# NickTravers/NeuralNetworkLibrary

Measured on AMD Instinct MI355X. Metric: ResNet-34 224x224 training throughput (Learner.train1minibatch, fwd+loss+bwd+optimizer), higher is better.
Workload: dtype f32; 1 GPU; DogsCats ResNet-34 classifier, 224x224, bs=64 per GPU, SGD momentum 0.9, fp32; global_batch=64, image_size=224, parallelism=dp1

## Files before the change

include/nnl.h:

```cpp
#ifndef NNL_H_
#define NNL_H_

#include <stddef.h>
#include <stdint.h>

#ifdef __cplusplus
extern "C" {
#endif

typedef enum {
  NNL_OK = 0,
  NNL_ERR_INVALID_ARG = -1,
  NNL_ERR_HIP = -2,
  NNL_ERR_UNSUPPORTED = -3,
  NNL_ERR_WORKSPACE = -4
} nnl_status_t;

int nnl_version(void);
const char* nnl_last_error(void);
int nnl_reload_env(void);

enum { NNL_PROF_CONV_FWD = 0, NNL_PROF_CONV_DGRAD = 1, NNL_PROF_CONV_WGRAD = 2, NNL_PROF_EMBDOT = 3,
       NNL_PROF_TABULAR = 4, NNL_PROF_RETINA_LOSS = 5, NNL_PROF_LSTM = 6, NNL_PROF_SOFTMAX_CE = 7,
       NNL_PROF_ELEMENTWISE = 8, NNL_PROF_GEMM = 9, NNL_PROF_OPTIM = 10, NNL_PROF_KINDS = 11 };
// ... 13 lines not shown
                       float* dU, float* dM, float* dbu, float* dbi, int64_t n, int64_t n_user,
                       int64_t n_item, int64_t D, int has_range, float lo, float hi, void* workspace, size_t workspace_bytes, void* stream);

typedef struct {
  int32_t N, H, W, C;
  int32_t K, R, S;
  int32_t stride, pad;
  int32_t P, Q;
} nnl_conv_geom_t;

size_t nnl_conv2d_fwd_workspace_bytes(const nnl_conv_geom_t* g);
int64_t nnl_conv2d_tile_counters(void);
int nnl_conv2d_fwd(const float* x, const float* w, const float* bias, float* y, const nnl_conv_geom_t* g,
                   int relu, void* workspace, size_t workspace_bytes, int32_t* tile_counters, float* bn_partials,
                   const float* bn_pivot, int32_t* bn_rows, void* stream);
int nnl_conv2d_fwd_add_up2(const float* x, const float* w, const float* bias, const float* small, float* y,
                           const nnl_conv_geom_t* g, void* stream);
int nnl_upsample2_bwd(const float* dy, float* dsmall, int64_t N, int64_t h, int64_t w, int64_t C, void* stream);
int nnl_conv2d_weight_transpose(const float* w, float* wt, int K, int R, int S, int C, void* stream);
typedef struct {
  const float* w;
  float* wt;
  int32_t K, RS, C, first_tile;
} nnl_wt_desc_t;
int nnl_conv2d_weight_transpose_multi(const nnl_wt_desc_t* desc, const int32_t* tile_tensor, int64_t n_tiles,
                                      double total_elems, void* stream);
size_t nnl_conv2d_dgrad_workspace_bytes(const nnl_conv_geom_t* g);
int nnl_conv2d_dgrad(const float* dy, const float* wt, float* dx, const nnl_conv_geom_t* g, const float* addend,
                     void* workspace, size_t workspace_bytes, int32_t* tile_counters, void* stream);
typedef struct {
// ... 37 lines not shown
int nnl_bn_fwd(const float* x, const float* gamma, const float* beta, const float* residual, float* y,
               float* save_mean, float* save_invstd, float* running_mean, float* running_var, int64_t rows,
               int64_t C, float eps, float momentum, int training, int relu, int64_t* num_batches_tracked,
               uint32_t* relu_mask, const float* ext_partials, int64_t ext_rows, const float* ext_pivot, float* pivot_out,
               void* workspace, size_t workspace_bytes, void* stream);
int nnl_bn_bwd(const float* dy, const float* y, const uint32_t* relu_mask, const float* x, const float* gamma,
               const float* mean, const float* invstd, float* dx, float* dres, float* dgamma, float* dbeta, int64_t rows,
               int64_t C, int training, int relu, void* workspace, size_t workspace_bytes, void* stream);

int nnl_bn_relu_maxpool_supported(int64_t C);
int nnl_bn_relu_maxpool_fwd(const float* x, const float* gamma, const float* beta, float* y, uint8_t* idx, float* save_mean,
                            float* save_invstd, float* save_scale, float* save_shift, float* running_mean, float* running_var,
                            int64_t N, int64_t H, int64_t W, int64_t C, int64_t P, int64_t Q, int ks, int stride, int pad, float eps,
                            float momentum, int training, int64_t* num_batches_tracked, void* workspace, size_t workspace_bytes,
                            void* stream);
int nnl_bn_relu_maxpool_bwd(const float* dpool, const float* y, const uint8_t* idx, const float* x, const float* gamma,
                            const float* beta, const float* mean, const float* invstd, const float* scale, const float* shift,
                            float* dx, float* dgamma, float* dbeta,
                            int64_t N, int64_t H, int64_t W, int64_t C, int64_t P, int64_t Q, int ks, int stride, int pad,
                            int training, void* workspace, size_t workspace_bytes, void* stream);

int nnl_debug_bn_plan(int64_t rows, int64_t C, int64_t N, int64_t H, int64_t W, int64_t P, int64_t Q, int32_t* out10);

int nnl_bn_sync_stats(const float* x, float* stats, int64_t rows, int64_t C, void* workspace, size_t workspace_bytes,
                      void* stream);
int nnl_bn_sync_fwd(const float* x, const float* all_stats, int world, const float* gamma, const float* beta,
                    const float* residual, float* y, float* save_mean, float* save_invstd, float* running_mean,
                    float* running_var, int64_t rows, int64_t C, float eps, float momentum, int relu,
                    int64_t* num_batches_tracked, uint32_t* relu_mask, void* workspace, size_t workspace_bytes, void* stream);
int nnl_bn_sync_bwd_reduce(const float* dy, const float* y, const uint32_t* relu_mask, const float* x, const float* mean,
// ... 239 lines not shown
```

neuralnetworklibrary_amd/_lib.py:

```python
import ctypes as C
import os

import torch

_HERE = os.path.dirname(os.path.abspath(__file__))
LIB_PATH = os.environ.get('NNL_LIB_PATH') or os.path.join(_HERE, 'libnnl_hip.so')

if not os.path.exists(LIB_PATH):
    raise ImportError(
        f"{LIB_PATH} not found: build it with `python -c 'import __graft_entry__ as g; g.build()'` "
        "(or `make -C neuralnetworklibrary_amd/csrc`). There is no CPU fallback for the HIP hot path.")

lib = C.CDLL(LIB_PATH)

c_p = C.c_void_p
i32, i64, f32, f64 = C.c_int32, C.c_int64, C.c_float, C.c_double
sz = C.c_size_t


class ConvGeom(C.Structure):
    _fields_ = [('N', i32), ('H', i32), ('W', i32), ('C', i32), ('K', i32), ('R', i32), ('S', i32),
                ('stride', i32), ('pad', i32), ('P', i32), ('Q', i32)]


# ... 21 lines not shown
    'nnl_conv2d_fwd_pre': (C.c_int, [c_p, c_p, c_p, c_p, C.POINTER(ConvGeom), C.c_int, c_p, sz, c_p, c_p, c_p, C.POINTER(i32), c_p, c_p]),
    'nnl_conv2d_dgrad_pre': (C.c_int, [c_p, c_p, c_p, C.POINTER(ConvGeom), c_p, c_p, sz, c_p, c_p, c_p]),
    'nnl_debug_conv_wino_workspace_bytes': (sz, [C.c_int] * 5),
    'nnl_debug_conv_wino_fwd': (C.c_int, [c_p] * 6 + [sz, c_p, C.c_long, c_p, c_p] + [C.c_int] * 7 + [c_p]),
    'nnl_debug_conv_wino2_workspace_bytes': (sz, [C.c_int] * 5),
    'nnl_debug_conv_wino2_fwd': (C.c_int, [c_p] * 6 + [sz, c_p, C.c_long, c_p, c_p] + [C.c_int] * 7 + [c_p]),
    'nnl_debug_conv_plan_times': (C.c_int, [C.c_int] * 5 + [C.POINTER(C.c_double)]),
    'nnl_debug_route_record': (C.c_int, [C.c_int]),
    'nnl_debug_route_collect': (C.c_int, [C.c_char_p, sz]),
    'nnl_conv2d_fwd': (C.c_int, [c_p, c_p, c_p, c_p, C.POINTER(ConvGeom), C.c_int, c_p, sz, c_p, c_p, c_p, C.POINTER(i32), c_p]),
    'nnl_conv2d_weight_transpose': (C.c_int, [c_p, c_p, C.c_int, C.c_int, C.c_int, C.c_int, c_p]),
    'nnl_conv2d_weight_transpose_multi': (C.c_int, [c_p, c_p, i64, f64, c_p]),
    'nnl_conv2d_dgrad': (C.c_int, [c_p, c_p, c_p, C.POINTER(ConvGeom), c_p, c_p, sz, c_p, c_p]),
    'nnl_conv2d_wgrad_workspace_bytes': (sz, [C.POINTER(ConvGeom)]),
    'nnl_conv2d_wgrad': (C.c_int, [c_p, c_p, c_p, C.POINTER(ConvGeom), c_p, sz, c_p]),
    'nnl_colsum_workspace_bytes': (sz, [i64, i64]),
    'nnl_colsum': (C.c_int, [c_p, c_p, i64, i64, c_p, sz, c_p]),
    'nnl_relu_gate_colsum': (C.c_int, [c_p, c_p, c_p, c_p, i64, i64, c_p, sz, c_p]),
    'nnl_conv2d_fwd_add_up2': (C.c_int, [c_p, c_p, c_p, c_p, c_p, C.POINTER(ConvGeom), c_p]),
    'nnl_upsample2_bwd': (C.c_int, [c_p, c_p, i64, i64, i64, i64, c_p]),
    'nnl_act_gate_colsum': (C.c_int, [c_p, c_p, c_p, c_p, i64, i64, C.c_int, c_p, sz, c_p]),
    'nnl_maxpool2d_fwd': (C.c_int, [c_p, c_p, c_p, i64, i64, i64, i64, i64, i64, C.c_int, C.c_int, C.c_int, c_p]),
    'nnl_maxpool2d_bwd': (C.c_int, [c_p, c_p, c_p, i64, i64, i64, i64, i64, i64, C.c_int, C.c_int, C.c_int, c_p]),
    'nnl_sum_tensors': (C.c_int, [c_p, C.c_int, c_p, i64, c_p]),
    'nnl_bn_relu_maxpool_supported': (C.c_int, [i64]),
    'nnl_bn_relu_maxpool_fwd': (C.c_int, [c_p, c_p, c_p, c_p, c_p, c_p, c_p, c_p, c_p, c_p, c_p, i64, i64, i64, i64, i64, i64,
                                          C.c_int, C.c_int, C.c_int, f32, f32, C.c_int, c_p, c_p, sz, c_p]),
    'nnl_bn_relu_maxpool_bwd': (C.c_int, [c_p, c_p, c_p, c_p, c_p, c_p, c_p, c_p, c_p, c_p, c_p, c_p, c_p, i64, i64, i64, i64, i64, i64,
                                          C.c_int, C.c_int, C.c_int, C.c_int, c_p, sz, c_p]),
    'nnl_concat_pool_fwd': (C.c_int, [c_p, c_p, c_p, i64, i64, i64, c_p]),
    'nnl_concat_pool_bwd': (C.c_int, [c_p, c_p, c_p, i64, i64, i64, c_p]),
    'nnl_gconv2d_fwd': (C.c_int, [c_p, c_p, c_p, c_p, i64, i64, i64, i64, i64, i64, C.c_int, C.c_int, C.c_int, C.c_int, c_p]),
    'nnl_gconv2d_dgrad': (C.c_int, [c_p, c_p, c_p, i64, i64, i64, i64, i64, i64, C.c_int, C.c_int, C.c_int, c_p]),
    'nnl_gconv2d_workspace_bytes': (sz, [i64, i64, i64, i64, i64, i64, C.c_int, C.c_int, C.c_int]),
    'nnl_gconv2d_wgrad': (C.c_int, [c_p, c_p, c_p, c_p, sz, i64, i64, i64, i64, i64, i64, C.c_int, C.c_int, C.c_int, c_p]),
    'nnl_se_squeeze': (C.c_int, [c_p, c_p, i64, i64, i64, c_p]),
    'nnl_se_excite_fwd': (C.c_int, [c_p, c_p, c_p, c_p, i64, i64, i64, c_p]),
    'nnl_se_excite_bwd': (C.c_int, [c_p, c_p, c_p, c_p, c_p, c_p, c_p, i64, i64, i64, c_p]),
    'nnl_se_squeeze_bwd': (C.c_int, [c_p, c_p, i64, i64, i64, c_p]),
    'nnl_bbox_decode': (C.c_int, [c_p, c_p, c_p, i64, i64, i64, c_p, c_p, f32, f32, f32, c_p, c_p, c_p, c_p, c_p, c_p]),
    'nnl_bbox_decode_window': (C.c_int, [c_p, c_p, c_p, i64, i64, i64, c_p, c_p, f32, f32, f32, f32, f32, c_p, c_p, c_p, c_p, c_p, c_p]),
    'nnl_nms_workspace_bytes': (sz, [i64, i64]),
# ... 142 lines not shown
```

neuralnetworklibrary_amd/csrc/batchnorm.hip:

```cpp
#include "nnl_common.h"

namespace {

typedef float f32x4 __attribute__((ext_vector_type(4)));

template <int VEC> struct VecT;
template <> struct VecT<4> { typedef f32x4 type; };
template <> struct VecT<1> { typedef float type; };

template <int VEC> __device__ __forceinline__ float vget(const typename VecT<VEC>::type& v, int i);
template <> __device__ __forceinline__ float vget<4>(const f32x4& v, int i) { return v[i]; }
template <> __device__ __forceinline__ float vget<1>(const float& v, int i) { return v; }
template <int VEC> __device__ __forceinline__ void vset(typename VecT<VEC>::type& v, int i, float x);
template <> __device__ __forceinline__ void vset<4>(f32x4& v, int i, float x) { v[i] = x; }
template <> __device__ __forceinline__ void vset<1>(float& v, int i, float x) { v = x; }

constexpr int kBlock = 256;
constexpr int kMaxRowBlocks = 1024;
constexpr float kCentreAbove = 16.f;
constexpr int kFinLanes = 64;

struct Shape {
  int L;
  int rpb;
// ... 799 lines not shown
  NNL_CHECK_ARG(P == (H + 2 * pad - ks) / stride + 1 && Q == (W + 2 * pad - ks) / stride + 1, "%s: P/Q do not match", who);
  NNL_CHECK_ARG(bnpool_ok(C), "%s: C=%ld needs C %% 4 == 0 and C/4 dividing 256", who, C);
  NNL_CHECK_ARG(N * H * W * C < (1L << 31) * 4, "%s: tensor too large", who);
  return NNL_OK;
}

}

extern "C" int nnl_bn_relu_maxpool_supported(int64_t C) { return bnpool_ok(C) ? 1 : 0; }

extern "C" int nnl_bn_relu_maxpool_fwd(const float* x, const float* gamma, const float* beta, float* y, uint8_t* idx,
                                       float* save_mean, float* save_invstd, float* save_scale, float* save_shift,
                                       float* running_mean, float* running_var, int64_t N, int64_t H, int64_t W, int64_t C,
                                       int64_t P, int64_t Q, int ks, int stride, int pad, float eps, float momentum, int training,
                                       int64_t* num_batches_tracked, void* workspace, size_t workspace_bytes, void* stream) {
  NNL_TRY(check_stem_geometry("bn_relu_maxpool_fwd", N, H, W, C, P, Q, ks, stride, pad));
  NNL_CHECK_ARG(x && y && idx && save_mean && save_invstd && save_scale && save_shift, "bn_relu_maxpool_fwd: null pointer");
  NNL_CHECK_ARG(training || (running_mean && running_var), "bn_relu_maxpool_fwd: eval mode needs running statistics");
  const long rows = (long)N * H * W, CG = C / 4;
  Workspace ws;
  NNL_TRY(bind_workspace(workspace, workspace_bytes, rows, C, "bn_relu_maxpool_fwd", ws));
  hipStream_t s = (hipStream_t)stream;
  NnlProfScope prof(NNL_PROF_ELEMENTWISE, s, (double)rows * C * (training ? 8.0 : 4.0) + (double)N * P * Q * C * 5.0);
  const ChannelStats cs{gamma, beta, save_mean, save_invstd, running_mean, running_var, save_scale, save_shift,  nullptr,
                         nullptr, num_batches_tracked, eps, momentum};
  NNL_TRY(launch_channel_affine(x, ws.part, cs, rows, C, training, s));
  const long total = (long)N * P * Q * CG;
  hipLaunchKernelGGL(bnpool_fwd_kernel, dim3((unsigned)nnl_cdiv(total, kBlock)), dim3(kBlock), 0, s, x, save_scale, save_shift, y, idx,
                     (int)N, (int)H, (int)W, (int)CG, (int)P, (int)Q, ks, stride, pad);
  NNL_CHECK_LAUNCH();
  return NNL_OK;
}

extern "C" int nnl_bn_relu_maxpool_bwd(const float* dpool, const float* y, const uint8_t* idx, const float* x, const float* gamma,
                                       const float* beta, const float* mean, const float* invstd, const float* scale,
                                       const float* shift, float* dx, float* dgamma, float* dbeta, int64_t N,
                                       int64_t H, int64_t W, int64_t C, int64_t P, int64_t Q, int ks, int stride, int pad,
                                       int training, void* workspace, size_t workspace_bytes, void* stream) {
  NNL_TRY(check_stem_geometry("bn_relu_maxpool_bwd", N, H, W, C, P, Q, ks, stride, pad));
  NNL_CHECK_ARG(dpool && idx && x && mean && invstd && scale && shift && dx, "bn_relu_maxpool_bwd: null pointer");
  const long rows = (long)N * H * W;
// ... 105 lines not shown
```

neuralnetworklibrary_amd/csrc/conv2d.hip:

```cpp
#include "igemm_kernels.h"
#include "igemm_taps.h"
#include "split_plan.h"
#include "wino.h"
#include "igemm_wgrad.h"
#include "igemm_wgrad2d.h"

#ifdef NNL_TAPS_TIMING
static void* g_wgrad_dbg = nullptr;
extern "C" void* nnl_debug_wgrad_stamps(void) { return g_wgrad_dbg; }
#endif

namespace {

int check_geom(const nnl_conv_geom_t* g, const char* who) {
  if (!g) return nnl_set_error(NNL_ERR_INVALID_ARG, "%s: null geometry", who);
  if (g->N <= 0 || g->H <= 0 || g->W <= 0 || g->C <= 0 || g->K <= 0 || g->R <= 0 || g->S <= 0 || g->stride <= 0 ||
      g->pad < 0)
    return nnl_set_error(NNL_ERR_INVALID_ARG, "%s: non-positive dimension", who);
  if (g->H + 2L * g->pad < g->R || g->W + 2L * g->pad < g->S)
    return nnl_set_error(NNL_ERR_INVALID_ARG, "%s: the %d x %d filter is larger than the padded input (%d x %d, pad %d)", who, g->R, g->S,
                         g->H, g->W, g->pad);
  const int P = (g->H + 2 * g->pad - g->R) / g->stride + 1, Q = (g->W + 2 * g->pad - g->S) / g->stride + 1;
  if (P != g->P || Q != g->Q || P <= 0 || Q <= 0)
    return nnl_set_error(NNL_ERR_INVALID_ARG, "%s: P,Q=(%d,%d) do not match the geometry (%d,%d)", who, g->P, g->Q, P, Q);
// ... 1017 lines not shown
  if (wgrad_wino_ok(g)) {
    const WgradPlan wp = plan_wgrad_wino(g);
    nnl_prof_exec_frac(1.0 / 1.5);
    int st2 = launch_wgrad_wino(dy, x, (float*)workspace, g, wp, s);
    if (st2) return st2;
    const long n4 = (long)g->K * 3 * (g->C / 4);
    NNL_ROUTE("wgrad_wino1d_finish");
    hipLaunchKernelGGL(wino_wgrad_finish_kernel, dim3((unsigned)nnl_cdiv(n4, 32L)), dim3(256), 0, s, (const float*)workspace, dw, n4,
                       g->C / 4, wp.splits, (long)g->K * 12 * (g->C / 4));
    NNL_CHECK_LAUNCH();
    return NNL_OK;
  }
  return launch_wgrad_direct(p, plan_wgrad(p.Mc, p.Nc, p.Kp), (float*)workspace, dw, s);
}

extern "C" size_t nnl_colsum_workspace_bytes(int64_t rows, int64_t cols) {
  if (rows <= 0 || cols <= 0) return 0;
  return (size_t)colsum_chunks(rows) * cols * sizeof(float);
}

extern "C" int nnl_act_gate_colsum(const float* dy, const float* y, float* g, float* colsum, int64_t rows, int64_t cols, int act,
                                   void* workspace, size_t workspace_bytes, void* stream) {
  NNL_CHECK_ARG(dy && y && g && rows > 0 && cols > 0 && cols < (1L << 30), "act_gate_colsum: bad argument");
  NNL_CHECK_ARG(act == 1 || act == 2, "act_gate_colsum: act must be 1 (ReLU) or 2 (sigmoid)");
  if (colsum != nullptr && (workspace == nullptr || workspace_bytes < nnl_colsum_workspace_bytes(rows, cols)))
    return nnl_set_error(NNL_ERR_WORKSPACE, "act_gate_colsum: workspace too small");
  hipStream_t s = (hipStream_t)stream;
  NnlProfScope prof(NNL_PROF_ELEMENTWISE, s, 12.0 * rows * cols);
  const int nchunk = colsum_chunks(rows);
  const long rpc = nnl_cdiv(nnl_cdiv(rows, nchunk), 4) * 4;
// ... 75 lines not shown
```

neuralnetworklibrary_amd/ops.py:

```python
import collections
import contextlib
import ctypes
import os
import weakref

import numpy as np
import torch

from . import _lib
from ._lib import check, lib, ptr, require_cuda, stream

__all__ = ['mse_loss', 'bce_with_logits', 'fbeta', 'scaled_sigmoid', 'embdotbias', 'index_error_flag', 'raise_if_index_error', 'conv2d', 'to_nhwc', 'from_nhwc', 'linear', 'bn_act', 'concat_pool2d', 'TabularPlan', 'tab_embed_concat', 'embedding_renorm_drop', 'retina_loss', 'image_aug', 'grouped_conv2d', 'se_excite']

_ERR_FLAGS = {}


def _flags(device):
    key = (device.type, device.index)
    if key not in _ERR_FLAGS:
        _ERR_FLAGS[key] = torch.zeros(2, dtype=torch.int32, device=device)
    return _ERR_FLAGS[key]


def index_error_flag(device):
# ... 565 lines not shown
        dxn += shortcut.view_as(dxn)
    give = st.give_slot
    if give is not None and not give.closed and st.c_in == g.C:
        give.tensor = dxn
        return None
    return from_nhwc(dxn[..., :st.c_in] if st.c_in != g.C else dxn)


def _conv_wgrad(st, xn, dy4, g4, K):
    dst = st.grad_dst
    if dst is not None and st.uses is not None and st.uses[0] == 1 and dst.dim() == 4 and g4.K == K and st.c_in == g4.C \
            and dst.permute(0, 2, 3, 1).is_contiguous() and tuple(dst.shape) == (g4.K, g4.C, g4.R, g4.S):
        dwn = dst.permute(0, 2, 3, 1)
    else:
        dwn = torch.empty((g4.K, g4.R, g4.S, g4.C), dtype=torch.float32, device=dy4.device)
    wsb = int(lib.nnl_conv2d_wgrad_workspace_bytes(g4))
    ws = _workspace(wsb, dy4.device, floor=True)
    check(lib.nnl_conv2d_wgrad(ptr(xn), ptr(dy4), ptr(dwn), g4, ptr(ws), wsb, stream()))
    dw = from_nhwc(dwn[:K, :, :, :st.c_in])
    wshape, wstride = st.w_layout
    if (g4.R == 1 and g4.S == 1 and wshape == tuple(dw.shape) and wstride != tuple(dw.stride()) and dw.is_contiguous(memory_format=torch.channels_last)
            and wstride[1] == 1 and wstride[0] == dw.shape[1]):
        dw = dw.as_strided(wshape, wstride)
    return dw


def _conv_bias_grad(dy4, g4, K):
    rows = g4.N * g4.P * g4.Q
    db_full = torch.empty(g4.K, dtype=torch.float32, device=dy4.device)
    cb = int(lib.nnl_colsum_workspace_bytes(rows, g4.K))
    cws = _workspace(cb, dy4.device, floor=True)
    check(lib.nnl_colsum(ptr(dy4), ptr(db_full), rows, g4.K, ptr(cws), cb, stream()))
    return db_full[:K]


class _Conv2d(torch.autograd.Function):

    @staticmethod
    def forward(ctx, x, weight, bias, stride, pad, relu, slot=None, bn_pivot=None, give_slot=None):
        require_cuda(x, weight, bias)
        xn, wn, b, g, y = _conv_operands(x, weight, bias, stride, pad)
        N, K = g.N, g.K
        ctx.st = _conv_state(x, weight, bias, g, relu, slot, give_slot)
        wsb = int(lib.nnl_conv2d_fwd_workspace_bytes(g))
        ws = _workspace(wsb, x.device)
        part, rows = None, _lib.i32(0)
        if bn_pivot is not None:
            part = torch.empty(((N * g.P * g.Q + 63) // 64) * K * 2, dtype=torch.float32, device=x.device)
        u = (_OPEN or _CLOSED).wino(wn.data_ptr(), 0, g)
        check(lib.nnl_conv2d_fwd_pre(ptr(xn), ptr(wn), ptr(b), ptr(y), g, int(relu), ptr(ws), wsb, ptr(_tile_counters(x.device) if wsb else None),
                                     ptr(part), ptr(bn_pivot), ctypes.byref(rows) if part is not None else None, ptr(u), stream()))
        if part is None or rows.value == 0:
            part = torch.empty(0, dtype=torch.float32, device=x.device)
        else:
            part = part[:rows.value * K * 2]
        ctx.mark_non_differentiable(part)
        ctx.set_materialize_grads(False)
        ctx.save_for_backward(xn, wn, y if relu else None)
        return from_nhwc(y), part

    @staticmethod
    def backward(ctx, dy, _dpart=None):
        xn, wn, y = ctx.saved_tensors
        return _conv_backward(ctx.st, xn, wn, y, dy, ctx.needs_input_grad[:3]) + (None,) * 6


# ... 328 lines not shown
        return from_nhwc(y)

    @staticmethod
    def backward(ctx, dy):
        (idx,) = ctx.saved_tensors
        N, H, W, C, P, Q, ksize, stride, pad = ctx.cfg
        dyn = to_nhwc(dy.float())
        dx = torch.empty(N, H, W, C, dtype=torch.float32, device=dy.device)
        check(lib.nnl_maxpool2d_bwd(ptr(dyn), ptr(idx), ptr(dx), N, H, W, C, P, Q, ksize, stride, pad, stream()))
        return from_nhwc(dx), None, None, None, None


class _BNReLUMaxPool(torch.autograd.Function):

    @staticmethod
    def forward(ctx, x, gamma, beta, running_mean, running_var, training, momentum, eps, nbt, ksize, stride, pad):
        require_cuda(x, gamma, beta)
        xn = to_nhwc(x.float())
        N, H, W, C = xn.shape
        P, Q = (H + 2 * pad - ksize) // stride + 1, (W + 2 * pad - ksize) // stride + 1
        dev = x.device
        y = torch.empty(N, P, Q, C, dtype=torch.float32, device=dev)
        idx = torch.empty(N, P, Q, C, dtype=torch.uint8, device=dev)
        stats = torch.empty(4, C, dtype=torch.float32, device=dev)
        wsb = int(lib.nnl_bn_workspace_bytes(N * H * W, C))
        ws = _workspace(wsb, dev)
        check(lib.nnl_bn_relu_maxpool_fwd(ptr(xn), ptr(gamma), ptr(beta), ptr(y), ptr(idx), ptr(stats[0]), ptr(stats[1]),
                                          ptr(stats[2]), ptr(stats[3]), ptr(running_mean), ptr(running_var), N, H, W, C, P, Q,
                                          ksize, stride, pad, float(eps), float(momentum), int(training), ptr(nbt), ptr(ws), wsb,
                                          stream()))
        ctx.save_for_backward(xn, idx, gamma, beta, stats, y)
        ctx.cfg = (N, H, W, C, P, Q, ksize, stride, pad, training)
        return from_nhwc(y)

    @staticmethod
    def backward(ctx, dy):
        xn, idx, gamma, beta, stats, y = ctx.saved_tensors
        N, H, W, C, P, Q, ksize, stride, pad, training = ctx.cfg
        dyn = to_nhwc(dy.float())
        dx = torch.empty_like(xn)
        dgamma = torch.empty(C, dtype=torch.float32, device=xn.device) if gamma is not None else None
        dbeta = torch.empty(C, dtype=torch.float32, device=xn.device) if gamma is not None else None
        wsb = int(lib.nnl_bn_workspace_bytes(N * H * W, C))
        ws = _workspace(wsb, xn.device)
        check(lib.nnl_bn_relu_maxpool_bwd(ptr(dyn), ptr(y), ptr(idx), ptr(xn), ptr(gamma), ptr(beta), ptr(stats[0]), ptr(stats[1]),
                                          ptr(stats[2]), ptr(stats[3]), ptr(dx), ptr(dgamma), ptr(dbeta), N, H, W, C, P, Q, ksize, stride, pad,
                                          int(training), ptr(ws), wsb, stream()))
        return (from_nhwc(dx), dgamma, dbeta) + (None,) * 9


def conv_bn_relu_maxpool(conv, bn, pool, x):
    k, s, p = pool.kernel_size, pool.stride, pool.padding
    fuse = (x.is_cuda and isinstance(pool, torch.nn.MaxPool2d) and all(isinstance(v, int) for v in (k, s, p))
            and pool.dilation == 1 and not pool.ceil_mode and not pool.return_indices and 2 * p <= k and k * k <= 255
            and not (bn.training and getattr(bn, 'nnl_sync', None) is not None)
            and (bn.running_mean is not None or bn.training)
            and not (bn.training and bn.track_running_stats and bn.momentum is None)
            and bool(lib.nnl_bn_relu_maxpool_supported(bn.num_features)))
    if not fuse:
        return pool(conv_bn_act(conv, bn, x, relu=True))
    y = conv(x)
    training, momentum, nbt, rmean, rvar = _bn_mode(bn)
    return _BNReLUMaxPool.apply(y, bn.weight, bn.bias, rmean, rvar, training, momentum, bn.eps, nbt, k, s, p)


def maxpool2d(x, ksize=3, stride=2, pad=1, ceil_mode=False):
    return _MaxPool2d.apply(x, int(ksize), int(stride), int(pad), bool(ceil_mode))


def _gconv_check(x_shape, w_shape, stride, pad, groups):
    if len(x_shape) != 4 or len(w_shape) != 4:
        raise NotImplementedError('grouped_conv2d: x %s and weight %s must be 4-D' % (tuple(x_shape), tuple(w_shape)))
    C, (K, Cg, R, S) = x_shape[1], w_shape
    if R != S or R not in (1, 3):
        raise NotImplementedError('grouped_conv2d: kernel_size %dx%d is not supported (1x1 or 3x3)' % (R, S))
    if stride not in (1, 2):
        raise NotImplementedError('grouped_conv2d: stride %r is not supported (1 or 2)' % (stride,))
    if pad not in (0, 1) or pad > R // 2:
# ... 841 lines not shown
```

Baseline: 5540 images/s.

## Add dedicated 7x7 stem conv kernels with fused BN statistics epilogue

Adds a specialized MFMA kernel for the 7x7 stride-2 stem convolution (C padded to 4, K multiple of 64), plus a slab-based wgrad kernel with a reduction pass. The forward kernel can emit per-channel BN partial sums, and the fused BN+ReLU+maxpool path now consumes those partials instead of re-reading the conv output to compute statistics. The goal is to replace the generic conv path for the stem and remove one full pass over the large stem activation. This adds complexity: a pivot tensor cached on the BN module, a skip during graph capture, and a dedicated code path whose numerics may differ slightly.

```diff
diff --git a/include/nnl.h b/include/nnl.h
--- a/include/nnl.h
+++ b/include/nnl.h
@@ -51,6 +51,12 @@
 int nnl_conv2d_fwd(const float* x, const float* w, const float* bias, float* y, const nnl_conv_geom_t* g,
                    int relu, void* workspace, size_t workspace_bytes, int32_t* tile_counters, float* bn_partials,
                    const float* bn_pivot, int32_t* bn_rows, void* stream);
+int nnl_stem7_supported(const nnl_conv_geom_t* g);
+int nnl_stem7_fwd(const float* x, const float* w, const float* bias, float* y, const nnl_conv_geom_t* g, int relu, float* bn_partials,
+                  const float* bn_pivot, int32_t* bn_rows, void* stream);
+size_t nnl_stem7_wgrad_workspace_bytes(const nnl_conv_geom_t* g);
+int nnl_stem7_wgrad(const float* x, const float* dy, float* dw, const nnl_conv_geom_t* g, void* workspace, size_t workspace_bytes,
+                    void* stream);
 int nnl_conv2d_fwd_add_up2(const float* x, const float* w, const float* bias, const float* small, float* y,
                            const nnl_conv_geom_t* g, void* stream);
 int nnl_upsample2_bwd(const float* dy, float* dsmall, int64_t N, int64_t h, int64_t w, int64_t C, void* stream);
@@ -118,6 +124,12 @@
                             int64_t N, int64_t H, int64_t W, int64_t C, int64_t P, int64_t Q, int ks, int stride, int pad, float eps,
                             float momentum, int training, int64_t* num_batches_tracked, void* workspace, size_t workspace_bytes,
                             void* stream);
+int nnl_bn_relu_maxpool_fwd_ext(const float* x, const float* gamma, const float* beta, float* y, uint8_t* idx, float* save_mean,
+                                float* save_invstd, float* save_scale, float* save_shift, float* running_mean, float* running_var,
+                                int64_t N, int64_t H, int64_t W, int64_t C, int64_t P, int64_t Q, int ks, int stride, int pad,
+                                float eps, float momentum, int training, int64_t* num_batches_tracked, const float* ext_partials,
+                                int64_t ext_rows, const float* ext_pivot, float* pivot_out, void* workspace, size_t workspace_bytes,
+                                void* stream);
 int nnl_bn_relu_maxpool_bwd(const float* dpool, const float* y, const uint8_t* idx, const float* x, const float* gamma,
                             const float* beta, const float* mean, const float* invstd, const float* scale, const float* shift,
                             float* dx, float* dgamma, float* dbeta,
diff --git a/neuralnetworklibrary_amd/_lib.py b/neuralnetworklibrary_amd/_lib.py
--- a/neuralnetworklibrary_amd/_lib.py
+++ b/neuralnetworklibrary_amd/_lib.py
@@ -59,6 +59,10 @@
     'nnl_conv2d_dgrad': (C.c_int, [c_p, c_p, c_p, C.POINTER(ConvGeom), c_p, c_p, sz, c_p, c_p]),
     'nnl_conv2d_wgrad_workspace_bytes': (sz, [C.POINTER(ConvGeom)]),
     'nnl_conv2d_wgrad': (C.c_int, [c_p, c_p, c_p, C.POINTER(ConvGeom), c_p, sz, c_p]),
+    'nnl_stem7_supported': (C.c_int, [C.POINTER(ConvGeom)]),
+    'nnl_stem7_fwd': (C.c_int, [c_p, c_p, c_p, c_p, C.POINTER(ConvGeom), C.c_int, c_p, c_p, C.POINTER(i32), c_p]),
+    'nnl_stem7_wgrad_workspace_bytes': (sz, [C.POINTER(ConvGeom)]),
+    'nnl_stem7_wgrad': (C.c_int, [c_p, c_p, c_p, C.POINTER(ConvGeom), c_p, sz, c_p]),
     'nnl_colsum_workspace_bytes': (sz, [i64, i64]),
     'nnl_colsum': (C.c_int, [c_p, c_p, i64, i64, c_p, sz, c_p]),
     'nnl_relu_gate_colsum': (C.c_int, [c_p, c_p, c_p, c_p, i64, i64, c_p, sz, c_p]),
@@ -71,6 +75,8 @@
     'nnl_bn_relu_maxpool_supported': (C.c_int, [i64]),
     'nnl_bn_relu_maxpool_fwd': (C.c_int, [c_p, c_p, c_p, c_p, c_p, c_p, c_p, c_p, c_p, c_p, c_p, i64, i64, i64, i64, i64, i64,
                                           C.c_int, C.c_int, C.c_int, f32, f32, C.c_int, c_p, c_p, sz, c_p]),
+    'nnl_bn_relu_maxpool_fwd_ext': (C.c_int, [c_p, c_p, c_p, c_p, c_p, c_p, c_p, c_p, c_p, c_p, c_p, i64, i64, i64, i64, i64, i64,
+                                              C.c_int, C.c_int, C.c_int, f32, f32, C.c_int, c_p, c_p, i64, c_p, c_p, c_p, sz, c_p]),
     'nnl_bn_relu_maxpool_bwd': (C.c_int, [c_p, c_p, c_p, c_p, c_p, c_p, c_p, c_p, c_p, c_p, c_p, c_p, c_p, i64, i64, i64, i64, i64, i64,
                                           C.c_int, C.c_int, C.c_int, C.c_int, c_p, sz, c_p]),
     'nnl_concat_pool_fwd': (C.c_int, [c_p, c_p, c_p, i64, i64, i64, c_p]),
diff --git a/neuralnetworklibrary_amd/csrc/batchnorm.hip b/neuralnetworklibrary_amd/csrc/batchnorm.hip
--- a/neuralnetworklibrary_amd/csrc/batchnorm.hip
+++ b/neuralnetworklibrary_amd/csrc/batchnorm.hip
@@ -837,6 +837,18 @@
                                        float* running_mean, float* running_var, int64_t N, int64_t H, int64_t W, int64_t C,
                                        int64_t P, int64_t Q, int ks, int stride, int pad, float eps, float momentum, int training,
                                        int64_t* num_batches_tracked, void* workspace, size_t workspace_bytes, void* stream) {
+  return nnl_bn_relu_maxpool_fwd_ext(x, gamma, beta, y, idx, save_mean, save_invstd, save_scale, save_shift, running_mean, running_var, N, H,
+                                     W, C, P, Q, ks, stride, pad, eps, momentum, training, num_batches_tracked, nullptr, 0, nullptr, nullptr,
+                                     workspace, workspace_bytes, stream);
+}
+
+extern "C" int nnl_bn_relu_maxpool_fwd_ext(const float* x, const float* gamma, const float* beta, float* y, uint8_t* idx,
+                                           float* save_mean, float* save_invstd, float* save_scale, float* save_shift,
+                                           float* running_mean, float* running_var, int64_t N, int64_t H, int64_t W, int64_t C,
+                                           int64_t P, int64_t Q, int ks, int stride, int pad, float eps, float momentum, int training,
+                                           int64_t* num_batches_tracked, const float* ext_partials, int64_t ext_rows,
+                                           const float* ext_pivot, float* pivot_out, void* workspace, size_t workspace_bytes,
+                                           void* stream) {
   NNL_TRY(check_stem_geometry("bn_relu_maxpool_fwd", N, H, W, C, P, Q, ks, stride, pad));
   NNL_CHECK_ARG(x && y && idx && save_mean && save_invstd && save_scale && save_shift, "bn_relu_maxpool_fwd: null pointer");
   NNL_CHECK_ARG(training || (running_mean && running_var), "bn_relu_maxpool_fwd: eval mode needs running statistics");
@@ -846,8 +858,11 @@
   hipStream_t s = (hipStream_t)stream;
   NnlProfScope prof(NNL_PROF_ELEMENTWISE, s, (double)rows * C * (training ? 8.0 : 4.0) + (double)N * P * Q * C * 5.0);
   const ChannelStats cs{gamma, beta, save_mean, save_invstd, running_mean, running_var, save_scale, save_shift,  nullptr,
-                         nullptr, num_batches_tracked, eps, momentum};
-  NNL_TRY(launch_channel_affine(x, ws.part, cs, rows, C, training, s));
+                        pivot_out, num_batches_tracked, eps, momentum};
+  if (training && ext_partials != nullptr && ext_rows > 0 && ext_pivot != nullptr)
+    NNL_TRY(launch_finalize(ext_pivot, ext_partials, (int)ext_rows, true, cs, rows, C, s));
+  else
+    NNL_TRY(launch_channel_affine(x, ws.part, cs, rows, C, training, s));
   const long total = (long)N * P * Q * CG;
   hipLaunchKernelGGL(bnpool_fwd_kernel, dim3((unsigned)nnl_cdiv(total, kBlock)), dim3(kBlock), 0, s, x, save_scale, save_shift, y, idx,
                      (int)N, (int)H, (int)W, (int)CG, (int)P, (int)Q, ks, stride, pad);
diff --git a/neuralnetworklibrary_amd/csrc/conv2d.hip b/neuralnetworklibrary_amd/csrc/conv2d.hip
--- a/neuralnetworklibrary_amd/csrc/conv2d.hip
+++ b/neuralnetworklibrary_amd/csrc/conv2d.hip
@@ -4,6 +4,7 @@
 #include "wino.h"
 #include "igemm_wgrad.h"
 #include "igemm_wgrad2d.h"
+#include "stem7.h"
 
 #ifdef NNL_TAPS_TIMING
 static void* g_wgrad_dbg = nullptr;
@@ -1055,6 +1056,46 @@
   return launch_wgrad_direct(p, plan_wgrad(p.Mc, p.Nc, p.Kp), (float*)workspace, dw, s);
 }
 
+extern "C" int nnl_stem7_supported(const nnl_conv_geom_t* g) { return g && check_geom(g, "stem7_supported") == NNL_OK && nnl_stem7_ok(g) ? 1 : 0; }
+
+extern "C" int nnl_stem7_fwd(const float* x, const float* w, const float* bias, float* y, const nnl_conv_geom_t* g, int relu,
+                             float* bn_partials, const float* bn_pivot, int32_t* bn_rows, void* stream) {
+  if (bn_rows) *bn_rows = 0;
+  int st = check_geom(g, "stem7_fwd");
+  if (st) return st;
+  NNL_CHECK_ARG(x && w && y, "stem7_fwd: null pointer");
+  NNL_CHECK_ARG(relu == 0 || relu == 1, "stem7_fwd: relu (activation) must be 0 none or 1 ReLU");
+  if (!nnl_stem7_ok(g))
+    return nnl_set_error(NNL_ERR_UNSUPPORTED, "stem7_fwd: needs a 7x7 / stride 2 / pad 3 filter, C == 4, K %% 64 == 0 and tensors below 2^31 bytes");
+  hipStream_t s = (hipStream_t)stream;
+  NnlProfScope prof(NNL_PROF_CONV_FWD, s, 2.0 * g->N * g->P * g->Q * (double)g->K * g->R * g->S * g->C);
+  nnl_prof_exec_frac(148.0 / 196.0);
+  const bool stats = bn_partials && bn_pivot && bn_rows;
+  st = nnl_stem7_fwd_launch(x, w, bias, y, g, relu, stats ? bn_partials : nullptr, bn_pivot, s);
+  if (st == NNL_OK && stats) *bn_rows = nnl_stem7_fwd_rows(g);
+  return st;
+}
+
+extern "C" size_t nnl_stem7_wgrad_workspace_bytes(const nnl_conv_geom_t* g) {
+  return nnl_stem7_supported(g) ? nnl_stem7_wgrad_slab_bytes(g) : 0;
+}
+
+extern "C" int nnl_stem7_wgrad(const float* x, const float* dy, float* dw, const nnl_conv_geom_t* g, void* workspace, size_t workspace_bytes,
+                               void* stream) {
+  int st = check_geom(g, "stem7_wgrad");
+  if (st) return st;
+  NNL_CHECK_ARG(x && dy && dw, "stem7_wgrad: null pointer");
+  if (!nnl_stem7_ok(g))
+    return nnl_set_error(NNL_ERR_UNSUPPORTED, "stem7_wgrad: needs a 7x7 / stride 2 / pad 3 filter, C == 4, K %% 64 == 0 and tensors below 2^31 bytes");
+  const size_t need = nnl_stem7_wgrad_slab_bytes(g);
+  if (workspace == nullptr || workspace_bytes < need)
+    return nnl_set_error(NNL_ERR_WORKSPACE, "stem7_wgrad: workspace %zu B < required %zu B", workspace_bytes, need);
+  hipStream_t s = (hipStream_t)stream;
+  NnlProfScope prof(NNL_PROF_CONV_WGRAD, s, 2.0 * g->N * g->P * g->Q * (double)g->K * g->R * g->S * g->C);
+  nnl_prof_exec_frac(160.0 / 196.0);
+  return nnl_stem7_wgrad_launch(x, dy, dw, g, (float*)workspace, s);
+}
+
 extern "C" size_t nnl_colsum_workspace_bytes(int64_t rows, int64_t cols) {
   if (rows <= 0 || cols <= 0) return 0;
   return (size_t)colsum_chunks(rows) * cols * sizeof(float);
diff --git a/neuralnetworklibrary_amd/csrc/stem7.h b/neuralnetworklibrary_amd/csrc/stem7.h
--- /dev/null
+++ b/neuralnetworklibrary_amd/csrc/stem7.h
@@ -0,0 +1,9 @@
+#pragma once
+#include "nnl_common.h"
+
+bool nnl_stem7_ok(const nnl_conv_geom_t* g);
+int nnl_stem7_fwd_rows(const nnl_conv_geom_t* g);
+int nnl_stem7_fwd_launch(const float* x, const float* w, const float* bias, float* y, const nnl_conv_geom_t* g, int relu, float* bn_part,
+                         const float* bn_pivot, hipStream_t s);
+size_t nnl_stem7_wgrad_slab_bytes(const nnl_conv_geom_t* g);
+int nnl_stem7_wgrad_launch(const float* x, const float* dy, float* dw, const nnl_conv_geom_t* g, float* ws, hipStream_t s);
diff --git a/neuralnetworklibrary_amd/csrc/stem7.hip b/neuralnetworklibrary_amd/csrc/stem7.hip
--- /dev/null
+++ b/neuralnetworklibrary_amd/csrc/stem7.hip
@@ -0,0 +1,396 @@
+#include "stem7.h"
+#include "split_tile.h"
+
+namespace {
+
+constexpr int kTR = 4, kTC = 16;
+constexpr int kPR = 2 * kTR + 5, kPC = 2 * kTC + 5;
+constexpr int kRS = 112;
+constexpr int kPatch = kPR * kRS;
+constexpr int kSteps = 74;
+constexpr int kOS = 68;
+constexpr int kMaxGroups = 512;
+
+struct Stem7Params {
+  const float* x;
+  const float* w;
+  float* y;
+  const float* bias;
+  float* bn_part;
+  const float* bn_pivot;
+  int N, H, W, P, Q, Nc;
+  int relu;
+  int n_pb, n_qb, n_blocks;
+};
+
+struct Slot { int off, rowpair, klo, khi; };
+__host__ __device__ constexpr Slot stem7_slot(int t) {
+  if (t < 70) return Slot{(t / 10) * kRS + 2 * (t % 10), 0, (t / 10) * 21 + 2 * (t % 10), (t / 10) * 21 + 2 * (t % 10) + 1};
+  if (t < 73) return Slot{2 * (t - 70) * kRS + 20, 1, 2 * (t - 70) * 21 + 20, (2 * (t - 70) + 1) * 21 + 20};
+  return Slot{6 * kRS + 20, 0, 6 * 21 + 20, -1};
+}
+__host__ __device__ constexpr int stem7_widx(int k) { return (k / 3) * 4 + k % 3; }
+
+struct PatchWalk {
+  int qb, pb, n;
+  int lr[2], lc[2];
+  bool ok[2];
+  __device__ __forceinline__ void init(int b0, int n_pb, int n_qb, int tid) {
+    qb = b0 % n_qb; pb = (b0 / n_qb) % n_pb; n = b0 / n_qb / n_pb;
+#pragma unroll
+    for (int u = 0; u < 2; ++u) {
+      const int e = tid + u * 256;
+      ok[u] = e < kPR * kPC;
+      lr[u] = e / kPC; lc[u] = e - lr[u] * kPC;
+    }
+  }
+  __device__ __forceinline__ void next(int n_pb, int n_qb) {
+    if (++qb == n_qb) { qb = 0; if (++pb == n_pb) { pb = 0; ++n; } }
+  }
+  __device__ __forceinline__ void load(const float* x, int H, int W, f32x4 (&v)[2]) const {
+    const int ih0 = pb * (2 * kTR) - 3, iw0 = qb * (2 * kTC) - 3;
+#pragma unroll
+    for (int u = 0; u < 2; ++u) {
+      const int ih = ih0 + lr[u], iw = iw0 + lc[u];
+      v[u] = f32x4{0.f, 0.f, 0.f, 0.f};
+      if (ok[u] && ih >= 0 && ih < H && iw >= 0 && iw < W) v[u] = *reinterpret_cast<const f32x4*>(x + (((long)n * H + ih) * W + iw) * 4);
+    }
+  }
+  __device__ __forceinline__ void store(float* patch, const f32x4 (&v)[2]) const {
+#pragma unroll
+    for (int u = 0; u < 2; ++u)
+      if (ok[u]) {
+        float* d = &patch[lr[u] * kRS + lc[u] * 3];
+        d[0] = v[u][0]; d[1] = v[u][1]; d[2] = v[u][2];
+      }
+  }
+};
+
+constexpr int kDepth = 6;
+typedef __attribute__((address_space(3))) float lds_float;
+__device__ __forceinline__ unsigned lds_addr(float* q) { return (unsigned)(uintptr_t)(lds_float*)q; }
+
+template <int T>
+__device__ __forceinline__ void a_issue(float (&ring)[kDepth], unsigned addr_a, unsigned addr_b) {
+  if constexpr (T < kSteps) {
+    constexpr Slot sl = stem7_slot(T);
+    asm volatile("ds_read_b32 %0, %1 offset:%2" : "=v"(ring[T % kDepth]) : "v"(sl.rowpair ? addr_b : addr_a), "n"(sl.off * 4) : "memory");
+  }
+}
+
+template <int T>
+__device__ __forceinline__ void a_steps(f32x16& acc, float (&ring)[kDepth], const float (&breg)[kSteps], unsigned addr_a, unsigned addr_b,
+                                        int hi) {
+  if constexpr (T < kSteps) {
+    constexpr int left = kSteps - 1 - T < kDepth - 1 ? kSteps - 1 - T : kDepth - 1;
+    asm volatile("s_waitcnt lgkmcnt(%1)" : "+v"(ring[T % kDepth]) : "n"(left));
+    float a = ring[T % kDepth];
+    if constexpr (stem7_slot(T).khi < 0) a = hi ? 0.f : a;
+    acc = __builtin_amdgcn_mfma_f32_32x32x2f32(a, breg[T], acc, 0, 0, 0);
+    a_issue<T + kDepth>(ring, addr_a, addr_b);
+    a_steps<T + 1>(acc, ring, breg, addr_a, addr_b, hi);
+  }
+}
+
+template <int T>
+__device__ __forceinline__ void a_prime(float (&ring)[kDepth], unsigned addr_a, unsigned addr_b) {
+  if constexpr (T < kDepth) {
+    a_issue<T>(ring, addr_a, addr_b);
+    a_prime<T + 1>(ring, addr_a, addr_b);
+  }
+}
+
+__global__ __launch_bounds__(256, 2) void stem7_fwd_kernel(const Stem7Params p) {
+  __shared__ float patch[2][kPatch];
+  __shared__ float outs[2][64 * kOS];
+  const int tid = threadIdx.x, lane = tid & 63, wave = tid >> 6;
+  const int hi = lane >> 5, li = lane & 31;
+  const int ph = wave & 1, chh = wave >> 1;
+  const int n0 = blockIdx.y * 64;
+
+  float breg[kSteps];
+  {
+    const float* wl = p.w + (long)(n0 + chh * 32 + li) * 196;
+#pragma unroll
+    for (int t = 0; t < kSteps; ++t) {
+      const Slot sl = stem7_slot(t);
+      const float wv = wl[hi && sl.khi >= 0 ? stem7_widx(sl.khi >= 0 ? sl.khi : 0) : stem7_widx(sl.klo)];
+      breg[t] = hi && sl.khi < 0 ? 0.f : wv;
+    }
+  }
+  const int pix = (2 * (2 * ph + (li >> 4))) * kRS + 6 * (li & 15);
+  const int base_a = pix + hi, base_b = pix + hi * kRS;
+
+  const int G = gridDim.x, g = blockIdx.x;
+  const int b0 = (int)((long)g * p.n_blocks / G), b1 = (int)((long)(g + 1) * p.n_blocks / G);
+  PatchWalk walk;
+  walk.init(b0, p.n_pb, p.n_qb, tid);
+
+  const int c4 = (tid & 15) * 4, epc = tid >> 4;
+  float fs1[4] = {0.f, 0.f, 0.f, 0.f}, fs2[4] = {0.f, 0.f, 0.f, 0.f};
+  f32x4 pv = {0.f, 0.f, 0.f, 0.f};
+  if (p.bn_part) pv = *reinterpret_cast<const f32x4*>(p.bn_pivot + n0 + c4);
+
+  f32x4 stage[2];
+  walk.load(p.x, p.H, p.W, stage);
+  walk.store(patch[0], stage);
+  __syncthreads();
+
+  for (int b = b0; b < b1; ++b) {
+    const int buf = (b - b0) & 1;
+    const int cn = walk.n, cp0 = walk.pb * kTR, cq0 = walk.qb * kTC;
+    walk.next(p.n_pb, p.n_qb);
+    if (b + 1 < b1) walk.load(p.x, p.H, p.W, stage);
+
+    f32x16 acc;
+#pragma unroll
+    for (int e = 0; e < 16; ++e) acc[e] = 0.f;
+    {
+      const unsigned addr_a = lds_addr(&patch[buf][base_a]), addr_b = lds_addr(&patch[buf][base_b]);
+      float ring[kDepth];
+      a_prime<0>(ring, addr_a, addr_b);
+      a_steps<0>(acc, ring, breg, addr_a, addr_b, hi);
+    }
+
+    float* os = outs[buf];
+#pragma unroll
+    for (int e = 0; e < 16; ++e) os[(ph * 32 + (e & 3) + 8 * (e >> 2) + 4 * hi) * kOS + chh * 32 + li] = acc[e];
+    if (b + 1 < b1) walk.store(patch[buf ^ 1], stage);
+    __syncthreads();
+
+    const int q = cq0 + epc;
+#pragma unroll
+    for (int e = 0; e < kTR; ++e) {
+      const int pr = cp0 + e;
+      if (pr < p.P && q < p.Q) {
+        f32x4 v = *reinterpret_cast<const f32x4*>(&os[(e * 16 + epc) * kOS + c4]);
+        const long o = (((long)cn * p.P + pr) * p.Q + q) * p.Nc + n0 + c4;
+        v = finish4<false>(v, p.bias, n0 + c4, nullptr, 0, p.relu);
+        *reinterpret_cast<f32x4*>(p.y + o) = v;
+        if (p.bn_part) {
+#pragma unroll
+          for (int c = 0; c < 4; ++c) { const float d = v[c] - pv[c]; fs1[c] += d; fs2[c] += d * d; }
+        }
+      }
+    }
+  }
+  bn_partials_write(p, fs1, fs2, outs[0], tid, (int)blockIdx.x, n0);
+}
+
+constexpr int kCols = 160, kColTiles = 5, kPairs = kTC / 2, kWReads = kPairs * kColTiles, kWDepth = 10;
+
+struct Stem7WgradParams {
+  const float* x;
+  const float* dy;
+  float* slabs;
+  int N, H, W, P, Q, Nc;
+  int n_pb, n_qb, n_blocks;
+};
+
+template <int U>
+__device__ __forceinline__ void w_issue(float (&ring)[kWDepth], const unsigned (&addr)[kColTiles]) {
+  if constexpr (U < kWReads)
+    asm volatile("ds_read_b32 %0, %1 offset:%2" : "=v"(ring[U % kWDepth]) : "v"(addr[U % kColTiles]), "n"((U / kColTiles) * 12 * 4) : "memory");
+}
+
+template <int U>
+__device__ __forceinline__ void w_prime(float (&ring)[kWDepth], const unsigned (&addr)[kColTiles]) {
+  if constexpr (U < kWDepth) {
+    w_issue<U>(ring, addr);
+    w_prime<U + 1>(ring, addr);
+  }
+}
+
+template <int U>
+__device__ __forceinline__ void w_steps(f32x16 (&acc)[2][kColTiles], float (&ring)[kWDepth], const float (&dyv)[kPairs][2],
+                                        const unsigned (&addr)[kColTiles]) {
+  if constexpr (U < kWReads) {
+    constexpr int left = kWReads - 1 - U < kWDepth - 1 ? kWReads - 1 - U : kWDepth - 1;
+    constexpr int pp = U / kColTiles, ct = U % kColTiles;
+    asm volatile("s_waitcnt lgkmcnt(%1)" : "+v"(ring[U % kWDepth]) : "n"(left));
+    const float b = ring[U % kWDepth];
+    acc[0][ct] = __builtin_amdgcn_mfma_f32_32x32x2f32(dyv[pp][0], b, acc[0][ct], 0, 0, 0);
+    acc[1][ct] = __builtin_amdgcn_mfma_f32_32x32x2f32(dyv[pp][1], b, acc[1][ct], 0, 0, 0);
+    w_issue<U + kWDepth>(ring, addr);
+    w_steps<U + 1>(acc, ring, dyv, addr);
+  }
+}
+
+__global__ __launch_bounds__(256, 2) void stem7_wgrad_kernel(const Stem7WgradParams p) {
+  __shared__ float patch[2][kPatch];
+  __shared__ float red[2 * kColTiles * 16 * 64];
+  const int tid = threadIdx.x, lane = tid & 63, wave = tid >> 6;
+  const int hi = lane >> 5, li = lane & 31;
+  const int n0 = blockIdx.y * 64;
+
+  int off[kColTiles];
+#pragma unroll
+  for (int ct = 0; ct < kColTiles; ++ct) {
+    const int col = ct * 32 + li;
+    off[ct] = 2 * wave * kRS + 6 * hi + (col < 147 ? (col / 21) * kRS + col % 21 : 0);
+  }
+
+  const int G = gridDim.x, g = blockIdx.x;
+  const int b0 = (int)((long)g * p.n_blocks / G), b1 = (int)((long)(g + 1) * p.n_blocks / G);
+  PatchWalk walk;
+  walk.init(b0, p.n_pb, p.n_qb, tid);
+
+  auto load_dy = [&](float (&v)[kPairs][2]) {
+    const int pr = walk.pb * kTR + wave;
+#pragma unroll
+    for (int pp = 0; pp < kPairs; ++pp) {
+      const int q = walk.qb * kTC + 2 * pp + hi;
+      const bool in = pr < p.P && q < p.Q;
+      const float* d = p.dy + (((long)walk.n * p.P + pr) * p.Q + q) * p.Nc + n0 + li;
+      v[pp][0] = in ? d[0] : 0.f;
+      v[pp][1] = in ? d[32] : 0.f;
+    }
+  };
+
+  f32x16 acc[2][kColTiles];
+#pragma unroll
+  for (int h = 0; h < 2; ++h)
+#pragma unroll
+    for (int ct = 0; ct < kColTiles; ++ct)
+#pragma unroll
+      for (int e = 0; e < 16; ++e) acc[h][ct][e] = 0.f;
+
+  f32x4 stage[2];
+  float dy_next[kPairs][2];
+  walk.load(p.x, p.H, p.W, stage);
+  load_dy(dy_next);
+  walk.store(patch[0], stage);
+  __syncthreads();
+
+  for (int b = b0; b < b1; ++b) {
+    const int buf = (b - b0) & 1;
+    float dyv[kPairs][2];
+#pragma unroll
+    for (int pp = 0; pp < kPairs; ++pp) { dyv[pp][0] = dy_next[pp][0]; dyv[pp][1] = dy_next[pp][1]; }
+    walk.next(p.n_pb, p.n_qb);
+    if (b + 1 < b1) {
+      walk.load(p.x, p.H, p.W, stage);
+      load_dy(dy_next);
+    }
+    {
+      unsigned addr[kColTiles];
+#pragma unroll
+      for (int ct = 0; ct < kColTiles; ++ct) addr[ct] = lds_addr(&patch[buf][off[ct]]);
+      float ring[kWDepth];
+      w_prime<0>(ring, addr);
+      w_steps<0>(acc, ring, dyv, addr);
+    }
+    if (b + 1 < b1) walk.store(patch[buf ^ 1], stage);
+    __syncthreads();
+  }
+
+  for (int turn = 3; turn >= 0; --turn) {
+    if (wave == turn) {
+#pragma unroll
+      for (int h = 0; h < 2; ++h)
+#pragma unroll
+        for (int ct = 0; ct < kColTiles; ++ct)
+#pragma unroll
+          for (int e = 0; e < 16; ++e) {
+            float* r = &red[((h * kColTiles + ct) * 16 + e) * 64 + lane];
+            if (turn < 3) acc[h][ct][e] = *r + acc[h][ct][e];
+            if (turn > 0) *r = acc[h][ct][e];
+          }
+    }
+    __syncthreads();
+  }
+  if (wave == 0) {
+    float* slab = p.slabs + ((long)blockIdx.x * p.Nc + n0) * kCols;
+#pragma unroll
+    for (int h = 0; h < 2; ++h)
+#pragma unroll
+      for (int ct = 0; ct < kColTiles; ++ct)
+        if (ct * 32 + li < 147) {
+#pragma unroll
+          for (int e = 0; e < 16; ++e) slab[(h * 32 + (e & 3) + 8 * (e >> 2) + 4 * hi) * kCols + ct * 32 + li] = acc[h][ct][e];
+        }
+  }
+}
+
+__global__ __launch_bounds__(256) void stem7_wgrad_reduce_kernel(const float* __restrict__ slabs, float* __restrict__ dw, int n_slabs, int K) {
+  __shared__ float part[8][32];
+  const int col = threadIdx.x & 31, sl = threadIdx.x >> 5;
+  const int o = blockIdx.x * 32 + col, total = K * 196;
+  const int ch = o / 196, rem = o - ch * 196, c = rem & 3;
+  float a = 0.f;
+  if (o < total && c < 3) {
+    const float* src = slabs + (long)ch * kCols + (rem >> 2) * 3 + c;
+    const long stride = (long)K * kCols;
+    int s = sl;
+    for (; s + 24 < n_slabs; s += 32) {
+      const float v0 = src[s * stride], v1 = src[(s + 8) * stride], v2 = src[(s + 16) * stride], v3 = src[(s + 24) * stride];
+      a += v0; a += v1; a += v2; a += v3;
+    }
+    for (; s < n_slabs; s += 8) a += src[s * stride];
+  }
+  part[sl][col] = a;
+  __syncthreads();
+  if (sl == 0 && o < total) {
+    float t = part[0][col];
+#pragma unroll
+    for (int l = 1; l < 8; ++l) t += part[l][col];
+    dw[o] = c < 3 ? t : 0.f;
+  }
+}
+
+Stem7Params stem7_params(const nnl_conv_geom_t* g) {
+  Stem7Params p{};
+  p.N = g->N; p.H = g->H; p.W = g->W; p.P = g->P; p.Q = g->Q; p.Nc = g->K;
+  p.n_pb = (int)nnl_cdiv(g->P, kTR); p.n_qb = (int)nnl_cdiv(g->Q, kTC);
+  p.n_blocks = g->N * p.n_pb * p.n_qb;
+  return p;
+}
+
+}
+
+bool nnl_stem7_ok(const nnl_conv_geom_t* g) {
+  return g->R == 7 && g->S == 7 && g->stride == 2 && g->pad == 3 && g->C == 4 && g->K % 64 == 0 &&
+         (long)g->N * g->H * g->W * g->C * 4 < (1L << 31) && (long)g->N * g->P * g->Q * g->K * 4 < (1L << 31);
+}
+
+int nnl_stem7_fwd_rows(const nnl_conv_geom_t* g) {
+  const long tiles = nnl_cdiv((long)g->N * g->P * g->Q, 64);
+  return (int)(tiles < kMaxGroups ? tiles : kMaxGroups);
+}
+
+int nnl_stem7_fwd_launch(const float* x, const float* w, const float* bias, float* y, const nnl_conv_geom_t* g, int relu, float* bn_part,
+                         const float* bn_pivot, hipStream_t s) {
+  Stem7Params p = stem7_params(g);
+  p.x = x; p.w = w; p.y = y; p.bias = bias; p.relu = relu;
+  p.bn_part = bn_part; p.bn_pivot = bn_pivot;
+  NNL_ROUTE("stem7:fwd");
+  hipLaunchKernelGGL(stem7_fwd_kernel, dim3(nnl_stem7_fwd_rows(g), g->K / 64), dim3(256), 0, s, p);
+  NNL_CHECK_LAUNCH();
+  return NNL_OK;
+}
+
+static int nnl_stem7_wgrad_slabs(const nnl_conv_geom_t* g) {
+  const long blocks = (long)g->N * nnl_cdiv(g->P, kTR) * nnl_cdiv(g->Q, kTC);
+  return (int)(blocks < kMaxGroups ? blocks : kMaxGroups);
+}
+
+size_t nnl_stem7_wgrad_slab_bytes(const nnl_conv_geom_t* g) {
+  return (size_t)nnl_stem7_wgrad_slabs(g) * g->K * kCols * sizeof(float);
+}
+
+int nnl_stem7_wgrad_launch(const float* x, const float* dy, float* dw, const nnl_conv_geom_t* g, float* ws, hipStream_t s) {
+  const Stem7Params q = stem7_params(g);
+  Stem7WgradParams p{};
+  p.x = x; p.dy = dy; p.slabs = ws;
+  p.N = q.N; p.H = q.H; p.W = q.W; p.P = q.P; p.Q = q.Q; p.Nc = q.Nc;
+  p.n_pb = q.n_pb; p.n_qb = q.n_qb; p.n_blocks = q.n_blocks;
+  const int slabs = nnl_stem7_wgrad_slabs(g);
+  NNL_ROUTE("stem7:wgrad@slabs=%d", slabs);
+  hipLaunchKernelGGL(stem7_wgrad_kernel, dim3(slabs, g->K / 64), dim3(256), 0, s, p);
+  NNL_CHECK_LAUNCH();
+  NNL_ROUTE("stem7:wgrad_reduce");
+  hipLaunchKernelGGL(stem7_wgrad_reduce_kernel, dim3((unsigned)nnl_cdiv((long)g->K * 196, 32)), dim3(256), 0, s, (const float*)ws, dw, slabs,
+                     g->K);
+  NNL_CHECK_LAUNCH();
+  return NNL_OK;
+}
diff --git a/neuralnetworklibrary_amd/ops.py b/neuralnetworklibrary_amd/ops.py
--- a/neuralnetworklibrary_amd/ops.py
+++ b/neuralnetworklibrary_amd/ops.py
@@ -603,9 +603,10 @@
         dwn = dst.permute(0, 2, 3, 1)
     else:
         dwn = torch.empty((g4.K, g4.R, g4.S, g4.C), dtype=torch.float32, device=dy4.device)
-    wsb = int(lib.nnl_conv2d_wgrad_workspace_bytes(g4))
+    stem = bool(lib.nnl_stem7_supported(g4))
+    wsb = int((lib.nnl_stem7_wgrad_workspace_bytes if stem else lib.nnl_conv2d_wgrad_workspace_bytes)(g4))
     ws = _workspace(wsb, dy4.device, floor=True)
-    check(lib.nnl_conv2d_wgrad(ptr(xn), ptr(dy4), ptr(dwn), g4, ptr(ws), wsb, stream()))
+    check((lib.nnl_stem7_wgrad if stem else lib.nnl_conv2d_wgrad)(ptr(xn), ptr(dy4), ptr(dwn), g4, ptr(ws), wsb, stream()))
     dw = from_nhwc(dwn[:K, :, :, :st.c_in])
     wshape, wstride = st.w_layout
     if (g4.R == 1 and g4.S == 1 and wshape == tuple(dw.shape) and wstride != tuple(dw.stride()) and dw.is_contiguous(memory_format=torch.channels_last)
@@ -636,9 +637,14 @@
         part, rows = None, _lib.i32(0)
         if bn_pivot is not None:
             part = torch.empty(((N * g.P * g.Q + 63) // 64) * K * 2, dtype=torch.float32, device=x.device)
-        u = (_OPEN or _CLOSED).wino(wn.data_ptr(), 0, g)
-        check(lib.nnl_conv2d_fwd_pre(ptr(xn), ptr(wn), ptr(b), ptr(y), g, int(relu), ptr(ws), wsb, ptr(_tile_counters(x.device) if wsb else None),
-                                     ptr(part), ptr(bn_pivot), ctypes.byref(rows) if part is not None else None, ptr(u), stream()))
+        if int(relu) != 2 and lib.nnl_stem7_supported(g):
+            check(lib.nnl_stem7_fwd(ptr(xn), ptr(wn), ptr(b), ptr(y), g, int(relu), ptr(part), ptr(bn_pivot),
+                                    ctypes.byref(rows) if part is not None else None, stream()))
+        else:
+            u = (_OPEN or _CLOSED).wino(wn.data_ptr(), 0, g)
+            check(lib.nnl_conv2d_fwd_pre(ptr(xn), ptr(wn), ptr(b), ptr(y), g, int(relu), ptr(ws), wsb,
+                                         ptr(_tile_counters(x.device) if wsb else None), ptr(part), ptr(bn_pivot),
+                                         ctypes.byref(rows) if part is not None else None, ptr(u), stream()))
         if part is None or rows.value == 0:
             part = torch.empty(0, dtype=torch.float32, device=x.device)
         else:
@@ -997,8 +1003,10 @@
 class _BNReLUMaxPool(torch.autograd.Function):
 
     @staticmethod
-    def forward(ctx, x, gamma, beta, running_mean, running_var, training, momentum, eps, nbt, ksize, stride, pad):
+    def forward(ctx, x, gamma, beta, running_mean, running_var, training, momentum, eps, nbt, ksize, stride, pad, ext_stats=None,
+                pivot_out=None):
         require_cuda(x, gamma, beta)
+        ext_part, ext_pivot = ext_stats if ext_stats is not None and ext_stats[0].numel() else (None, None)
         xn = to_nhwc(x.float())
         N, H, W, C = xn.shape
         P, Q = (H + 2 * pad - ksize) // stride + 1, (W + 2 * pad - ksize) // stride + 1
@@ -1008,10 +1016,11 @@
         stats = torch.empty(4, C, dtype=torch.float32, device=dev)
         wsb = int(lib.nnl_bn_workspace_bytes(N * H * W, C))
         ws = _workspace(wsb, dev)
-        check(lib.nnl_bn_relu_maxpool_fwd(ptr(xn), ptr(gamma), ptr(beta), ptr(y), ptr(idx), ptr(stats[0]), ptr(stats[1]),
-                                          ptr(stats[2]), ptr(stats[3]), ptr(running_mean), ptr(running_var), N, H, W, C, P, Q,
-                                          ksize, stride, pad, float(eps), float(momentum), int(training), ptr(nbt), ptr(ws), wsb,
-                                          stream()))
+        check(lib.nnl_bn_relu_maxpool_fwd_ext(ptr(xn), ptr(gamma), ptr(beta), ptr(y), ptr(idx), ptr(stats[0]), ptr(stats[1]),
+                                              ptr(stats[2]), ptr(stats[3]), ptr(running_mean), ptr(running_var), N, H, W, C, P, Q,
+                                              ksize, stride, pad, float(eps), float(momentum), int(training), ptr(nbt), ptr(ext_part),
+                                              0 if ext_part is None else ext_part.numel() // (2 * C), ptr(ext_pivot), ptr(pivot_out),
+                                              ptr(ws), wsb, stream()))
         ctx.save_for_backward(xn, idx, gamma, beta, stats, y)
         ctx.cfg = (N, H, W, C, P, Q, ksize, stride, pad, training)
         return from_nhwc(y)
@@ -1029,7 +1038,7 @@
         check(lib.nnl_bn_relu_maxpool_bwd(ptr(dyn), ptr(y), ptr(idx), ptr(xn), ptr(gamma), ptr(beta), ptr(stats[0]), ptr(stats[1]),
                                           ptr(stats[2]), ptr(stats[3]), ptr(dx), ptr(dgamma), ptr(dbeta), N, H, W, C, P, Q, ksize, stride, pad,
                                           int(training), ptr(ws), wsb, stream()))
-        return (from_nhwc(dx), dgamma, dbeta) + (None,) * 9
+        return (from_nhwc(dx), dgamma, dbeta) + (None,) * 11
 
 
 def conv_bn_relu_maxpool(conv, bn, pool, x):
@@ -1042,9 +1051,25 @@
             and bool(lib.nnl_bn_relu_maxpool_supported(bn.num_features)))
     if not fuse:
         return pool(conv_bn_act(conv, bn, x, relu=True))
-    y = conv(x)
     training, momentum, nbt, rmean, rvar = _bn_mode(bn)
-    return _BNReLUMaxPool.apply(y, bn.weight, bn.bias, rmean, rvar, training, momentum, bn.eps, nbt, k, s, p)
+
+    def tail(y, ext_stats=None, pivot_out=None):
+        return _BNReLUMaxPool.apply(y, bn.weight, bn.bias, rmean, rvar, training, momentum, bn.eps, nbt, k, s, p, ext_stats, pivot_out)
+    epi = (bn.training and bn.track_running_stats and bn.running_mean is not None and getattr(conv, 'nnl_hip_conv', False)
+           and conv.bias is None and not conv.fuse_relu and conv.dilation == (1, 1) and conv.groups == 1
+           and conv.stride[0] == conv.stride[1] and conv.padding[0] == conv.padding[1] and conv.padding_mode == 'zeros'
+           and torch.is_grad_enabled() and os.environ.get('NNL_BN_EPI_STATS', '1') != '0')
+    if not epi:
+        return tail(conv(x))
+    pivot = getattr(bn, '_nnl_pivot', None)
+    if pivot is None or pivot.device != x.device or pivot.numel() != bn.num_features:
+        if torch.cuda.is_current_stream_capturing():
+            return tail(conv(x))
+        pivot = torch.empty(bn.num_features, dtype=torch.float32, device=x.device)
+        object.__setattr__(bn, '_nnl_pivot', pivot)
+        return tail(conv(x), pivot_out=pivot)
+    y, part = conv2d_with_bn_stats(x, conv.weight, None, conv.stride[0], conv.padding[0], pivot)
+    return tail(y, ext_stats=(part, pivot), pivot_out=pivot)
 
 
 def maxpool2d(x, ksize=3, stride=2, pad=1, ceil_mode=False):
```

New measurement: 5628 images/s, median of 6. 1.02x the previous value.
